# NVlabs/sionna

Measured on NVIDIA H100. Metric: coded bits/s, LDPC5G n=8448 k=4224 BP-20 decode, higher is better.
Workload: dtype f32

## Files before the change

### sionna_b200/csrc/ldpc_bp_qc.cu

```cuda
#include <algorithm>
#include <climits>
#include <iterator>
#include <numeric>
#include <vector>
#include "sb_common.h"
#include "sb_math.h"
#include "sb_math2.cuh"
#include "ldpc_graph.h"
#include "ldpc_rules.cuh"

namespace {

constexpr int kLoop = INT_MAX;
constexpr int kRowMax[] = {kLoop, 20, 12, 8, 4};
constexpr int kColCut = 7, kColFused = 10;
constexpr int kColMax[] = {kLoop, 32, 20, 12, 8, 4, 2, kLoop, 12, 4, 1};
constexpr int kRowClasses = (int)std::size(kRowMax);
constexpr int kColClasses = (int)std::size(kColMax);

constexpr bool decreasing(const int* m, int lo, int hi) {
    for (int k = lo + 1; k < hi; ++k)
        if (m[k] >= m[k - 1]) return false;
    return true;
}
static_assert(decreasing(kRowMax, 0, kRowClasses), "row class bounds must decrease");
static_assert(decreasing(kColMax, 0, kColCut) && decreasing(kColMax, kColCut, kColFused), "column class bounds must decrease");
static_assert(kColFused == kColClasses - 1 && kColMax[kColFused] == 1, "the fused class holds degree-1 columns only");

constexpr int degree_class(const int* m, int lo, int hi, int d) {
    int k = hi - 1;
    while (k > lo && d > m[k]) --k;
    return k;
}

struct QcParams {
    int Z, n_rows, n_cols, nnz, N, E, E_alloc, n_in, n_out;
    int row_cls_end[kRowClasses];
    int col_cls_end[kColClasses];
    int row_cls_mod[kRowClasses];
    int col_cls_mod[kColClasses];
    const int4* row_info;
    const int4* col_info;
    const int2* col_edge;
    const int* in_idx;
    const int* out_pos;
    const int* slot_of_edge;
    const float* llr;
    float* out;
    float* state_out;
    long long B;
    int num_iter, hard_out, use_tma;
    int early;
    int* iters_out;
    const int2* row_edge;
    int tab_rep;
    float offset, llr_max;
};


#define SB_PHI_HI 16.635532f
#define SB_PHI_ZERO 14.7117348f
template <class LT, class Probe>
__device__ __forceinline__ uint2 phi_pass1_pair(unsigned b0, unsigned b1, float& P, const LT& lt, Probe probe) {
    const float a0 = __uint_as_float(b0 & 0x7fffffffu), a1 = __uint_as_float(b1 & 0x7fffffffu);
    const float2 p = sb_phif2(make_float2(a0, a1), lt);
    probe(a0, a1);
    P = __fadd_rn(P, p.x);
    P = __fadd_rn(P, p.y);
    return make_uint2(__float_as_uint(p.x) | (b0 & 0x80000000u), __float_as_uint(p.y) | (b1 & 0x80000000u));
}
template <class LT>
__device__ __forceinline__ unsigned phi_pass1(unsigned b0, float& P, const LT& lt) {
    const float p = sb_phif_s(__uint_as_float(b0 & 0x7fffffffu), lt);
    P = __fadd_rn(P, p);
    return __float_as_uint(p) | (b0 & 0x80000000u);
}
template <class LT>
__device__ __forceinline__ uint2 phi_pass2_pair(unsigned w0, unsigned w1, float P, unsigned par, float clip, const LT& lt) {
    const float2 m = fadd2(make_float2(__uint_as_float(w0 | 0x80000000u), __uint_as_float(w1 | 0x80000000u)),
                           make_float2(P, P));
    const float2 y = sb_phif2(m, lt);
    return make_uint2(__float_as_uint(fminf(y.x, clip)) | ((w0 ^ par) & 0x80000000u),
                      __float_as_uint(fminf(y.y, clip)) | ((w1 ^ par) & 0x80000000u));
}
template <class LT>
__device__ __forceinline__ unsigned phi_pass2(unsigned w0, float P, unsigned par, float clip, const LT& lt) {
    const float y = sb_phif_s(__fadd_rn(__uint_as_float(w0 | 0x80000000u), P), lt);
    return __float_as_uint(fminf(y, clip)) | ((w0 ^ par) & 0x80000000u);
}
__device__ __forceinline__ unsigned ldw(const float* q) { return __float_as_uint(*q); }
__device__ __forceinline__ void stw(float* q, unsigned w) { *q = __uint_as_float(w); }

template <class LT>
__device__ __noinline__ void cn_phi_qc(float* pm, int Z, int deg, float clip, int* sat_flag, LT lt) {
    const unsigned am = __activemask();
    float P = 0.f;
    unsigned par = 0;
    int l = 0;
#pragma unroll 2
    for (; l + 1 < deg; l += 2) {
        float* q0 = pm + l * Z;
        float* q1 = q0 + Z;
        const unsigned b0 = ldw(q0), b1 = ldw(q1);
        par ^= b0 ^ b1;
        const uint2 w = phi_pass1_pair(b0, b1, P, lt, [&](float a0, float a1) {
            if (l == 0 && __all_sync(am, a0 >= SB_PHI_HI && a1 >= SB_PHI_HI)) *sat_flag = 1;
        });
        stw(q0, w.x);
        stw(q1, w.y);
    }
    if (l < deg) {
        float* q0 = pm + l * Z;
        const unsigned b0 = ldw(q0);
        par ^= b0;
        stw(q0, phi_pass1(b0, P, lt));
    }
    par &= 0x80000000u;
    l = 0;
#pragma unroll 2
    for (; l + 1 < deg; l += 2) {
        float* q0 = pm + l * Z;
        float* q1 = q0 + Z;
        const uint2 y = phi_pass2_pair(ldw(q0), ldw(q1), P, par, clip, lt);
        stw(q0, y.x);
        stw(q1, y.y);
    }
    if (l < deg) stw(pm + l * Z, phi_pass2(ldw(pm + l * Z), P, par, clip, lt));
}

__device__ __forceinline__ unsigned vote_sign(unsigned S, int l, unsigned par) { return ((S >> l) << 31) ^ par; }

__device__ __forceinline__ void vote_store_fast(float* pm, int Z, int deg, unsigned S, unsigned y, unsigned ylast) {
    const unsigned par = (unsigned)__popc(S) << 31;
    for (int l = 0; l < deg - 1; ++l) stw(pm + l * Z, y | vote_sign(S, l, par));
    stw(pm + (deg - 1) * Z, ylast | vote_sign(S, deg - 1, par));
}

template <class LT>
__device__ __noinline__ void cn_vote_row(float* pm, int Z, int deg, unsigned U, unsigned S, unsigned last, float clip,
                                         unsigned ylast, LT lt) {
    if (!(U & ~(1u << (deg - 1)))) {
        const float pl = sb_phif_s(__uint_as_float(last & 0x7fffffffu), lt);
        vote_store_fast(pm, Z, deg, S, __float_as_uint(fminf(sb_phif_s(pl, lt), clip)), ylast);
        return;
    }
    const unsigned par = (unsigned)__popc(S) << 31;
    float P = 0.f;
    unsigned u = U;
    for (; u & (u - 1); u &= u - 1) {
        float* q0 = pm + (__ffs(u) - 1) * Z;
        u &= u - 1;
        float* q1 = pm + (__ffs(u) - 1) * Z;
        const uint2 w = phi_pass1_pair(ldw(q0), ldw(q1), P, lt, [](float, float) {});
        stw(q0, w.x);
        stw(q1, w.y);
    }
    if (u) {
        float* q0 = pm + (__ffs(u) - 1) * Z;
        stw(q0, phi_pass1(ldw(q0), P, lt));
    }
    const unsigned rest = ~U & (0xffffffffu >> (32 - deg));
    if (rest) {
        const unsigned y = __float_as_uint(fminf(sb_phif_s(P, lt), clip));
        for (unsigned r = rest; r; r &= r - 1) {
            const int l = __ffs(r) - 1;
            stw(pm + l * Z, y | vote_sign(S, l, par));
        }
    }
    for (u = U; u & (u - 1); u &= u - 1) {
        float* q0 = pm + (__ffs(u) - 1) * Z;
        u &= u - 1;
        float* q1 = pm + (__ffs(u) - 1) * Z;
        const uint2 y = phi_pass2_pair(ldw(q0), ldw(q1), P, par, clip, lt);
        stw(q0, y.x);
        stw(q1, y.y);
    }
    if (u) {
        float* q0 = pm + (__ffs(u) - 1) * Z;
        stw(q0, phi_pass2(ldw(q0), P, par, clip, lt));
    }
}

template <int D, class LT>
__device__ __forceinline__ void cn_phi_qc_reg(float* pm, int Z, float clip, int* sat_flag, const LT& lt) {
    const unsigned am = __activemask();
    unsigned w[D];
    float P = 0.f;
    unsigned par = 0;
#pragma unroll
    for (int l = 0; l + 1 < D; l += 2) {
        const unsigned b0 = ldw(pm + l * Z), b1 = ldw(pm + (l + 1) * Z);
        par ^= b0 ^ b1;
        const uint2 q = phi_pass1_pair(b0, b1, P, lt, [&](float a0, float a1) {
            if (l == 0 && __all_sync(am, a0 >= SB_PHI_HI && a1 >= SB_PHI_HI)) *sat_flag = 1;
        });
        w[l] = q.x;
        w[l + 1] = q.y;
    }
    if (D & 1) {
        const unsigned b0 = ldw(pm + (D - 1) * Z);
        par ^= b0;
        w[D - 1] = phi_pass1(b0, P, lt);
    }
    par &= 0x80000000u;
#pragma unroll
    for (int l = 0; l + 1 < D; l += 2) {
        const uint2 y = phi_pass2_pair(w[l], w[l + 1], P, par, clip, lt);
        stw(pm + l * Z, y.x);
        stw(pm + (l + 1) * Z, y.y);
    }
    if (D & 1) stw(pm + (D - 1) * Z, phi_pass2(w[D - 1], P, par, clip, lt));
}

template <class LT, int... DS>
__device__ __forceinline__ bool cn_phi_reg_of(float* pm, int Z, int deg, float clip, int* sat_flag, const LT& lt) {
    return ((deg == DS && (cn_phi_qc_reg<DS, LT>(pm, Z, clip, sat_flag, lt), true)) || ...);
}

template <int CLS, class LT>
__device__ __forceinline__ void cn_phi_dispatch(float* pm, int Z, int deg, float clip, int* sat_flag, const LT& lt) {
    if (CLS == 4 && cn_phi_reg_of<LT, 3, 4>(pm, Z, deg, clip, sat_flag, lt)) return;
    if (CLS == 3 && cn_phi_reg_of<LT, 5, 6, 7, 8>(pm, Z, deg, clip, sat_flag, lt)) return;
    cn_phi_qc<LT>(pm, Z, deg, clip, sat_flag, lt);
}

struct StrideEdges {
    float* pm;
    int Z;
    __device__ __forceinline__ float in(int l) const { return pm[l * Z]; }
    __device__ __forceinline__ void out(int l, float v) const { pm[l * Z] = v; }
    __device__ __forceinline__ float staged(int l) const { return pm[l * Z]; }
};

__device__ __forceinline__ float2 minsum_mags(float m1, float m2, int deg, float clip, float offset) {
    float min_e = (m2 == m1) ? m1 : __fadd_rn(__fsub_rn(m2, m1), m1);
    if (deg == 1) min_e = __fadd_rn(100000.f, m1);
    return make_float2(fminf(fmaxf(__fsub_rn(m1, offset), 0.f), clip), fminf(fmaxf(__fsub_rn(min_e, offset), 0.f), clip));
}
__device__ __forceinline__ float minsum_msg(float v, float m1, float2 o, unsigned par) {
    const float mag = (fabsf(v) == m1) ? o.y : o.x;
    return __uint_as_float(__float_as_uint(mag) | ((__float_as_uint(v) ^ par) & 0x80000000u));
}
template <int DMAX, bool EXACT>
__device__ __forceinline__ void cn_minsum_qc(float* pm, int Z, int deg, float clip, float offset) {
    float x[DMAX];
    float m1 = INFINITY, m2 = INFINITY;
    unsigned par = 0;
#pragma unroll
    for (int l = 0; l < DMAX; ++l) {
        float v = INFINITY;
        if (EXACT || l < deg) v = pm[l * Z];
        x[l] = v;
        float a = fabsf(v);
        m2 = fminf(m2, fmaxf(m1, a));
        m1 = fminf(m1, a);
        par ^= __float_as_uint(v);
    }
    par &= 0x80000000u;
    const float2 o = minsum_mags(m1, m2, deg, clip, offset);
#pragma unroll
    for (int l = 0; l < DMAX; ++l) {
        const float y = minsum_msg(x[l], m1, o, par);
        if (EXACT || l < deg) pm[l * Z] = y;
    }
}

__device__ __forceinline__ void cn_minsum_qc_loop(float* pm, int Z, int deg, float clip, float offset) {
    float m1 = INFINITY, m2 = INFINITY;
    unsigned par = 0;
    for (int l = 0; l < deg; ++l) {
        float v = pm[l * Z];
        float a = fabsf(v);
        m2 = fminf(m2, fmaxf(m1, a));
        m1 = fminf(m1, a);
        par ^= __float_as_uint(v);
    }
    par &= 0x80000000u;
    const float2 o = minsum_mags(m1, m2, deg, clip, offset);
    for (int l = 0; l < deg; ++l) pm[l * Z] = minsum_msg(pm[l * Z], m1, o, par);
}

template <int RULE, int CLS, class LT>
__device__ __forceinline__ void cn_qc(float* pm, int Z, int deg, float clip, float offset, int* sat_flag, const LT& lt) {
    if constexpr (RULE == SB_CN_BOXPLUS_PHI) {
        cn_phi_dispatch<CLS, LT>(pm, Z, deg, clip, sat_flag, lt);
    } else if constexpr (RULE == SB_CN_BOXPLUS) {
        cn_tanh(StrideEdges{pm, Z}, deg, clip);
    } else {
        constexpr int D = kRowMax[CLS];
        const float off = (RULE == SB_CN_MINSUM) ? 0.f : offset;
        if constexpr (D == kLoop) {
            cn_minsum_qc_loop(pm, Z, deg, clip, off);
        } else if constexpr (CLS == 4) {
            if (deg == 3) cn_minsum_qc<3, true>(pm, Z, deg, clip, off);
            else if (deg == 4) cn_minsum_qc<4, true>(pm, Z, deg, clip, off);
            else cn_minsum_qc<D, false>(pm, Z, deg, clip, off);
        } else if constexpr (CLS == 3) {
            if (deg == 5) cn_minsum_qc<5, true>(pm, Z, deg, clip, off);
            else if (deg == 6) cn_minsum_qc<6, true>(pm, Z, deg, clip, off);
            else if (deg == 7) cn_minsum_qc<7, true>(pm, Z, deg, clip, off);
            else cn_minsum_qc<D, true>(pm, Z, deg, clip, off);
        } else if constexpr (CLS == 2) {
            if (deg == 9) cn_minsum_qc<9, true>(pm, Z, deg, clip, off);
            else if (deg == 10) cn_minsum_qc<10, true>(pm, Z, deg, clip, off);
            else cn_minsum_qc<D, false>(pm, Z, deg, clip, off);
        } else {
            if (deg == 19) cn_minsum_qc<19, true>(pm, Z, deg, clip, off);
            else cn_minsum_qc<D, false>(pm, Z, deg, clip, off);
        }
    }
}

__device__ __forceinline__ float lds_f32(uint32_t a) {
    float v;
    asm volatile("ld.shared.f32 %0, [%1];" : "=f"(v) : "r"(a));
    return v;
}
__device__ __forceinline__ void sts_f32(uint32_t a, float v) {
    asm volatile("st.shared.f32 [%0], %1;" ::"r"(a), "f"(v) : "memory");
}
__device__ __forceinline__ int2 lds_i2(uint32_t a) {
    int2 v;
    asm volatile("ld.shared.v2.s32 {%0, %1}, [%2];" : "=r"(v.x), "=r"(v.y) : "r"(a));
    return v;
}

template <int DMAX, bool CHECK, bool KEEPM, int MODE, bool EXACT = false>
__device__ __forceinline__ float vn_qc(uint32_t msg_s, uint32_t ce_s, int deg, int j4, int Z4, float llr, float clip) {
    uint32_t addr[DMAX];
    float m[KEEPM ? DMAX : 1];
    bool on[DMAX];
    float acc = 0.f;
#pragma unroll
    for (int k = 0; k < DMAX; ++k) {
        int2 e = make_int2(0, 0);
        if (EXACT || k < deg) e = lds_i2(ce_s + 8 * k);
        int t = j4 - (e.y & 0xffff);
        t += (t >> 31) & Z4;
        bool ok = EXACT || ((k < deg) && (!CHECK || t < (int)((unsigned)e.y >> 16)));
        on[k] = ok;
        addr[k] = msg_s + e.x + t;
        float v = 0.f;
        if (MODE == 0) {
            if (ok) v = lds_f32(addr[k]);
            if (ok) acc = __fadd_rn(acc, v);
        }
        if (KEEPM) m[KEEPM ? k : 0] = v;
    }
    float x_tot = __fadd_rn(acc, llr);
    const float init = __fadd_rn(llr, 0.f);
#pragma unroll
    for (int k = 0; k < DMAX; ++k) {
        if (MODE == 1) {
            if (on[k]) sts_f32(addr[k], init);
        } else {
            float v = 0.f;
            if (KEEPM) v = m[KEEPM ? k : 0];
            else if (on[k]) v = lds_f32(addr[k]);
            float y = clipf(__fadd_rn(-v, x_tot), clip);
            if (on[k]) sts_f32(addr[k], y);
        }
    }
    return x_tot;
}

template <int MODE>
__device__ __forceinline__ float vn_qc_loop(uint32_t msg_s, uint32_t ce_s, int deg, int j4, int Z4, float llr, float clip) {
    float acc = 0.f;
    if (MODE == 0)
        for (int k = 0; k < deg; ++k) {
            int2 e = lds_i2(ce_s + 8 * k);
            int t = j4 - (e.y & 0xffff);
            t += (t >> 31) & Z4;
            if (t < (int)((unsigned)e.y >> 16)) acc = __fadd_rn(acc, lds_f32(msg_s + e.x + t));
        }
    float x_tot = __fadd_rn(acc, llr);
    for (int k = 0; k < deg; ++k) {
        int2 e = lds_i2(ce_s + 8 * k);
        int t = j4 - (e.y & 0xffff);
        t += (t >> 31) & Z4;
        if (t < (int)((unsigned)e.y >> 16)) {
            uint32_t a = msg_s + e.x + t;
            sts_f32(a, (MODE == 1) ? __fadd_rn(llr, 0.f) : clipf(__fadd_rn(-lds_f32(a), x_tot), clip));
        }
    }
    return x_tot;
}

template <int MODE, int CLS, bool EX>
__device__ __forceinline__ float vn_cls(uint32_t msgb, uint32_t ce, int deg, int j4, int Z4, float llr, float clip) {
    constexpr int D = kColMax[CLS];
    if constexpr (D == kLoop) {
        return vn_qc_loop<MODE>(msgb, ce, deg, j4, Z4, llr, clip);
    } else if constexpr (CLS >= kColCut) {
        return vn_qc<D, true, true, MODE>(msgb, ce, deg, j4, Z4, llr, clip);
    } else if constexpr (D > 12) {
        return vn_qc<D, false, false, MODE>(msgb, ce, deg, j4, Z4, llr, clip);
    } else {
        if constexpr (CLS == 3) {
            if (EX && deg == 9) return vn_qc<9, false, true, MODE, true>(msgb, ce, deg, j4, Z4, llr, clip);
            if (EX && deg == 10) return vn_qc<10, false, true, MODE, true>(msgb, ce, deg, j4, Z4, llr, clip);
            if (EX && deg == 11) return vn_qc<11, false, true, MODE, true>(msgb, ce, deg, j4, Z4, llr, clip);
        } else if constexpr (CLS == 4) {
            if (EX && deg == 5) return vn_qc<5, false, true, MODE, true>(msgb, ce, deg, j4, Z4, llr, clip);
            if (EX && deg == 6) return vn_qc<6, false, true, MODE, true>(msgb, ce, deg, j4, Z4, llr, clip);
            if (EX && deg == 7) return vn_qc<7, false, true, MODE, true>(msgb, ce, deg, j4, Z4, llr, clip);
        } else if constexpr (CLS == 5) {
            if (EX && deg == 3) return vn_qc<3, false, true, MODE, true>(msgb, ce, deg, j4, Z4, llr, clip);
        } else {
            if (EX && deg == 1) return vn_qc<1, false, true, MODE, true>(msgb, ce, deg, j4, Z4, llr, clip);
        }
        return vn_qc<D, false, true, MODE, EX>(msgb, ce, deg, j4, Z4, llr, clip);
    }
}

struct WarpCtx {
    int G, grp, lane_i;
};

__device__ __forceinline__ int first_of(int start, int start_mod, const WarpCtx& w) {
    return start + (w.grp - start_mod + (w.grp < start_mod ? w.G : 0));
}

__device__ __forceinline__ void fused_vn(const QcParams& p, float* q, float c2v, int fw, int lane_i, const float* llr_s,
                                         float clip, unsigned char* hd) {
    int s = fw >> 16, vb = fw & 0xffff;
    int j = lane_i + s;
    j -= (j >= p.Z) ? p.Z : 0;
    float x_tot = __fadd_rn(__fadd_rn(0.f, c2v), llr_s[vb * p.Z + j]);
    *q = clipf(__fadd_rn(-c2v, x_tot), clip);
    if (hd) hd[vb * p.Z + j] = 0.f >= x_tot ? 1 : 0;
}

template <int RULE, int CLS, class LT>
__device__ __forceinline__ void cn_class(const QcParams& p, const WarpCtx& w, float* msg, const float* llr_s,
                                         const int4* s_row, int start, int end, float clip, bool fuse, int* sat_flag,
                                         const LT& lt, unsigned char* hd) {
    for (int rr = first_of(start, p.row_cls_mod[CLS], w); rr < end; rr += w.G) {
        int4 ri = s_row[rr];
        if (w.lane_i < ri.z) {
            float* pm = msg + ri.x * p.Z + w.lane_i;
            cn_qc<RULE, CLS, LT>(pm, p.Z, ri.y, clip, p.offset, sat_flag, lt);
            if (fuse && ri.w >= 0) {
                float* q = pm + (ri.y - 1) * p.Z;
                fused_vn(p, q, *q, ri.w, w.lane_i, llr_s, clip, hd);
            }
        }
    }
}

template <int RULE, class LT>
__device__ __forceinline__ void cn_all(const QcParams& p, const WarpCtx& w, float* msg, const float* llr_s,
                                       const int4* s_row, float clip, bool fuse, int* sat_flag, const LT& lt,
                                       unsigned char* hd) {
    const int* re = p.row_cls_end;
    cn_class<RULE, 0, LT>(p, w, msg, llr_s, s_row, 0, re[0], clip, fuse, sat_flag, lt, hd);
    cn_class<RULE, 1, LT>(p, w, msg, llr_s, s_row, re[0], re[1], clip, fuse, sat_flag, lt, hd);
    cn_class<RULE, 2, LT>(p, w, msg, llr_s, s_row, re[1], re[2], clip, fuse, sat_flag, lt, hd);
    cn_class<RULE, 3, LT>(p, w, msg, llr_s, s_row, re[2], re[3], clip, fuse, sat_flag, lt, hd);
    cn_class<RULE, 4, LT>(p, w, msg, llr_s, s_row, re[3], re[4], clip, fuse, sat_flag, lt, hd);
}

struct VoteRow {
    float* pm;
    int deg;
    bool act;
    unsigned own, S, last;
};

__device__ __forceinline__ VoteRow vote_row(float* msg, int4 ri, const WarpCtx& w, int Z) {
    VoteRow r;
    r.pm = msg + ri.x * Z + w.lane_i;
    r.deg = ri.y <= 32 ? ri.y : 0;
    r.act = w.lane_i < ri.z && r.deg > 0;
    r.own = r.S = r.last = 0;
    if (r.act) {
        r.last = ldw(r.pm + (r.deg - 1) * Z);
        r.own = fabsf(__uint_as_float(r.last)) < SB_PHI_ZERO ? 1u : 0u;
        r.S = r.last >> 31;
    }
    return r;
}

__device__ __forceinline__ void vote_read(VoteRow& r, int l, int o) {
    if (r.act && l < r.deg - 1) {
        const unsigned b = ldw(r.pm + o);
        r.own = __funnelshift_l(fabsf(__uint_as_float(b)) < SB_PHI_ZERO ? 0x80000000u : 0u, r.own, 1);
        r.S = __funnelshift_l(b, r.S, 1);
    }
}

template <class LT>
__device__ __forceinline__ void cn_vote_pass(const QcParams& p, const WarpCtx& w, float* msg, const float* llr_s,
                                             const int4* s_row, float clip, bool fuse, float phi_max, int* sat_flag,
                                             const LT& lt, unsigned char* hd) {
    const int Z = p.Z;
    const unsigned ylast = __float_as_uint(fminf(phi_max, clip));
    for (int rr = w.grp; rr < p.n_rows; rr += w.G) {
        const int4 ri = s_row[rr];
        VoteRow r = vote_row(msg, ri, w, Z);
        for (int l = r.deg - 2, o = l * Z; l >= 0; --l, o -= Z) vote_read(r, l, o);
        const unsigned U = __reduce_or_sync(0xffffffffu, r.own);
        if (r.act) cn_vote_row<LT>(r.pm, Z, r.deg, U, r.S, r.last, clip, ylast, lt);
        if (ri.y > 32 && w.lane_i < ri.z) cn_phi_qc<LT>(r.pm, Z, ri.y, clip, sat_flag, lt);
        if (fuse && ri.w >= 0 && w.lane_i < ri.z) {
            float* q = r.pm + (ri.y - 1) * Z;
            fused_vn(p, q, *q, ri.w, w.lane_i, llr_s, clip, hd);
        }
    }
}

__device__ __forceinline__ void syndrome_pass(const QcParams& p, const WarpCtx& w, const int4* s_row,
                                              const unsigned char* hd, int* unsat) {
    for (int rr = w.grp; rr < p.n_rows; rr += w.G) {
        const int4 ri = s_row[rr];
        if (w.lane_i < ri.z) {
            unsigned par = 0;
            for (int l = 0; l < ri.y; ++l) {
                const int2 e = __ldg(p.row_edge + ri.x + l);
                int j = w.lane_i + e.y;
                j -= (j >= p.Z) ? p.Z : 0;
                par ^= hd[e.x + j];
            }
            if (par) *unsat = 1;
        }
    }
}

template <int MODE, int CLS, bool EX>
__device__ __forceinline__ void vn_class(const QcParams& p, const WarpCtx& w, uint32_t msgb, const float* llr_s,
                                         const int4* s_col, uint32_t s_ce, int start, int end, float clip,
                                         bool final_pass, long long b, unsigned char* hd) {
    for (int cc = first_of(start, p.col_cls_mod[CLS], w); cc < end; cc += w.G) {
        int4 ci = s_col[cc];
        if (w.lane_i < ci.z) {
            int v = ci.w + w.lane_i;
            float x_tot = vn_cls<MODE, CLS, EX>(msgb, s_ce + 8 * ci.x, ci.y, 4 * w.lane_i, 4 * p.Z, llr_s[v], clip);
            if (MODE == 0 && hd) hd[v] = 0.f >= x_tot ? 1 : 0;
            if (MODE == 0 && final_pass) {
                int o = p.out_pos[v];
                if (o >= 0) {
                    x_tot = clipf(x_tot, clip);
                    p.out[(size_t)b * p.n_out + o] = decoder_out(x_tot, p.hard_out);
                }
            }
        }
    }
}

template <int MODE, bool EX>
__device__ __forceinline__ void vn_all(const QcParams& p, const WarpCtx& w, uint32_t msgb, const float* llr_s,
                                       const int4* s_col, uint32_t s_ce, float clip, bool final_pass,
                                       bool with_fused, long long b, unsigned char* hd = nullptr) {
    const int* ce = p.col_cls_end;
    vn_class<MODE, 0, EX>(p, w, msgb, llr_s, s_col, s_ce, 0, ce[0], clip, final_pass, b, hd);
    vn_class<MODE, 1, EX>(p, w, msgb, llr_s, s_col, s_ce, ce[0], ce[1], clip, final_pass, b, hd);
    vn_class<MODE, 2, EX>(p, w, msgb, llr_s, s_col, s_ce, ce[1], ce[2], clip, final_pass, b, hd);
    vn_class<MODE, 3, EX>(p, w, msgb, llr_s, s_col, s_ce, ce[2], ce[3], clip, final_pass, b, hd);
    vn_class<MODE, 4, EX>(p, w, msgb, llr_s, s_col, s_ce, ce[3], ce[4], clip, final_pass, b, hd);
    vn_class<MODE, 5, EX>(p, w, msgb, llr_s, s_col, s_ce, ce[4], ce[5], clip, final_pass, b, hd);
    vn_class<MODE, 6, EX>(p, w, msgb, llr_s, s_col, s_ce, ce[5], ce[6], clip, final_pass, b, hd);
    vn_class<MODE, 7, EX>(p, w, msgb, llr_s, s_col, s_ce, ce[6], ce[7], clip, final_pass, b, hd);
    vn_class<MODE, 8, EX>(p, w, msgb, llr_s, s_col, s_ce, ce[7], ce[8], clip, final_pass, b, hd);
    vn_class<MODE, 9, EX>(p, w, msgb, llr_s, s_col, s_ce, ce[8], ce[9], clip, final_pass, b, hd);
    if (with_fused) vn_class<MODE, 10, EX>(p, w, msgb, llr_s, s_col, s_ce, ce[9], ce[10], clip, final_pass, b, hd);
}

constexpr int kQcThreads = 768;

template <int RULE, int REP, bool EARLY>
__global__ void __launch_bounds__(kQcThreads, 1) ldpc_bp_qc_kernel(const __grid_constant__ QcParams p) {
    const int T = blockDim.x, tid = threadIdx.x, lane = tid & 31, warp = tid >> 5, W = T >> 5;
    const int Z = p.Z, N = p.N, Zb = (Z + 31) >> 5;
    unsigned char* const smem_raw = sb_smem + (RULE == SB_CN_BOXPLUS_PHI ? LogTab<REP>::bytes : 0);
    const int off_llr = p.E_alloc * 4;
    const int off_col = (off_llr + N * 4 + 15) & ~15;
    const int off_row = off_col + p.n_cols * 16;
    const int off_ce = off_row + p.n_rows * 16;
    const int off_bar = (off_ce + p.nnz * 8 + 15) & ~15;
    float* msg = reinterpret_cast<float*>(smem_raw);
    float* llr_s = reinterpret_cast<float*>(smem_raw + off_llr);
    int4* s_col = reinterpret_cast<int4*>(smem_raw + off_col);
    int4* s_row = reinterpret_cast<int4*>(smem_raw + off_row);
    int2* s_ce_p = reinterpret_cast<int2*>(smem_raw + off_ce);
    uint64_t* bar = reinterpret_cast<uint64_t*>(smem_raw + off_bar);
    int* sat_flag = reinterpret_cast<int*>(smem_raw + off_bar + 8);
    int* unsat = reinterpret_cast<int*>(smem_raw + off_bar + 12);
    unsigned char* hd = EARLY ? smem_raw + off_bar + 16 : nullptr;
    const uint32_t msgb = smem_u32(smem_raw);
    const uint32_t s_ce = msgb + off_ce;
    WarpCtx w;
    w.G = W / Zb;
    w.grp = warp / Zb;
    w.lane_i = (warp - w.grp * Zb) * 32 + lane;

    for (int i = tid; i < p.n_cols; i += T) s_col[i] = p.col_info[i];
    for (int i = tid; i < p.n_rows; i += T) s_row[i] = p.row_info[i];
    for (int i = tid; i < p.nnz; i += T) s_ce_p[i] = p.col_edge[i];
    const LogTab<REP> lt(lane);
    if (RULE == SB_CN_BOXPLUS_PHI) LogTab<REP>::fill(tid, T);
    if (p.use_tma && tid == 0) mbar_init(bar);
    __syncthreads();

    const float clip = p.llr_max;
    const float phi_max = sb_phif(0.f);
    uint32_t tma_phase = 0;

    for (long long b = blockIdx.x; b < p.B; b += gridDim.x) {
        load_channel_llr(llr_s, p.llr + (size_t)b * p.n_in, p.in_idx, N, p.n_in, clip, p.use_tma, msg, bar, tma_phase,
                         tid, T);
        __syncthreads();
        if (tid == 0) *sat_flag = 0;
        vn_all<1, true>(p, w, msgb, llr_s, s_col, s_ce, clip, false, true, b);
        __syncthreads();
        if (p.num_iter == 0) {
            for (int v = tid; v < N; v += T) {
                int o = p.out_pos[v];
                if (o >= 0) p.out[(size_t)b * p.n_out + o] = decoder_out(llr_s[v], p.hard_out);
            }
        }
        int limit = p.num_iter;
        for (int it = 0; it < limit; ++it) {
            if (EARLY && it > 0 && it < limit - 1) {
                if (tid == 0) *unsat = 0;
                __syncthreads();
                syndrome_pass(p, w, s_row, hd, unsat);
                __syncthreads();
                if (*unsat == 0) limit = it + 1;
            }
            const bool final_pass = it == limit - 1;
            const bool sc = *sat_flag != 0;
            if (final_pass && tid == 0 && p.use_tma && b + gridDim.x < p.B)
                asm volatile("cp.async.bulk.prefetch.L2.global [%0], %1;" ::"l"(p.llr + (size_t)(b + gridDim.x) * p.n_in),
                             "r"((uint32_t)p.n_in * 4u) : "memory");
            if constexpr (RULE == SB_CN_BOXPLUS_PHI) {
                if (sc) cn_vote_pass(p, w, msg, llr_s, s_row, clip, !final_pass, phi_max, sat_flag, lt, hd);
                else cn_all<RULE>(p, w, msg, llr_s, s_row, clip, !final_pass, sat_flag, lt, hd);
            } else {
                cn_all<RULE>(p, w, msg, llr_s, s_row, clip, !final_pass, sat_flag, lt, hd);
            }
            __syncthreads();
            vn_all<0, true>(p, w, msgb, llr_s, s_col, s_ce, clip, final_pass, final_pass, b, hd);
            __syncthreads();
        }
        if (EARLY && p.iters_out && tid == 0) p.iters_out[b] = limit;
        if (p.state_out) {
            store_state(p.state_out + (size_t)b * p.E, msg, p.slot_of_edge, p.E, tid, T);
            __syncthreads();
        }
    }
}

size_t qc_smem_bytes(const sb_ldpc_graph* g, int tab_rep, int early = 0) {
    return (early ? (size_t)g->N + 16 : 0) + ((size_t)g->qc_nnz * g->qc_Z + g->N) * 4 + 16 + (size_t)g->qc_cols * 16 + (size_t)g->qc_rows * 16 +
           (size_t)g->qc_nnz * 8 + 16 + 16 + (size_t)tab_rep * SB_LOGTAB_N * 8;
}

int qc_ensure_uploaded(sb_ldpc_graph* g) {
    if (g->qc_uploaded) return SB_OK;
    int rc;
    if ((rc = sb_upload(&g->d_qc_row_info, g->qc_row_info))) return rc;
    if ((rc = sb_upload(&g->d_qc_col_info, g->qc_col_info))) return rc;
    if ((rc = sb_upload(&g->d_qc_col_edge, g->qc_col_edge))) return rc;
    if ((rc = sb_upload(&g->d_qc_in_idx, g->qc_in_idx))) return rc;
    if ((rc = sb_upload(&g->d_qc_out_pos, g->qc_out_pos))) return rc;
    if ((rc = sb_upload(&g->d_qc_slot_of_edge, g->qc_slot_of_edge))) return rc;
    if ((rc = sb_upload(&g->d_qc_row_edge, g->qc_row_edge))) return rc;
    g->qc_uploaded = true;
    return SB_OK;
}

template <int RULE, bool EARLY>
int launch_qc(const sb_ldpc_graph* g, const QcParams& p, int threads, size_t smem, cudaStream_t stream) {
    auto kern = ldpc_bp_qc_kernel<RULE, 16, EARLY>;
    if constexpr (RULE == SB_CN_BOXPLUS_PHI) {
        if (p.tab_rep == 8) kern = ldpc_bp_qc_kernel<RULE, 8, EARLY>;
        if (p.tab_rep == 1) kern = ldpc_bp_qc_kernel<RULE, 1, EARLY>;
    }
    return sb_launch_decoder(kern, p, g, threads, smem, LLONG_MAX, stream, "sb_ldpc_decode(qc)");
}

}

void sb_qc_free_device(sb_ldpc_graph* g) {
    if (!g->qc_uploaded) return;
    cudaFree(g->d_qc_row_info); cudaFree(g->d_qc_col_info); cudaFree(g->d_qc_col_edge); cudaFree(g->d_qc_in_idx);
    cudaFree(g->d_qc_out_pos); cudaFree(g->d_qc_slot_of_edge); cudaFree(g->d_qc_row_edge);
    g->qc_uploaded = false;
}

extern "C" int sb_ldpc_graph_set_qc(sb_ldpc_graph* g, int32_t Z, int32_t n_entries, const int32_t* base_row,
                                    const int32_t* base_col, const int32_t* shift) {
    SB_CHECK_ARG(g && Z > 0 && Z <= 16383 && n_entries > 0 && base_row && base_col && shift, "sb_ldpc_graph_set_qc: bad arguments");
    SB_CHECK_ARG((int)g->h_cn.size() == g->E, "sb_ldpc_graph_set_qc: handle holds no edge list");
    SB_CHECK_ARG(!g->ref_order, "sb_ldpc_graph_set_qc: the QC kernel sums in ascending neighbour order; graphs created with "
                                "sb_ldpc_graph_create_ordered stay on the generic kernel");
    const int C = g->C, N = g->N, E = g->E;
    const int n_rows = (C + Z - 1) / Z, n_cols = (N + Z - 1) / Z;
    auto zrow = [&](int r) { return std::min(Z, C - r * Z); };
    auto zcol = [&](int c) { return std::min(Z, N - c * Z); };
    struct Ent { int r, c, s; };
    std::vector<Ent> ents;
    for (int k = 0; k < n_entries; ++k) {
        if (base_row[k] < 0 || base_col[k] < 0 || shift[k] < 0) { sb_set_error("sb_ldpc_graph_set_qc: negative entry"); return SB_EINVAL; }
        if (base_row[k] >= n_rows || base_col[k] >= n_cols) continue;
        ents.push_back({base_row[k], base_col[k], shift[k] % Z});
    }
    std::vector<long long> keys(E);
    for (int e = 0; e < E; ++e) keys[e] = ((long long)g->h_cn[e] << 32) | (unsigned)g->h_vn[e];
    std::sort(keys.begin(), keys.end());
    long long total = 0;
    for (const Ent& en : ents)
        for (int i = 0; i < zrow(en.r); ++i) {
            int j = (i + en.s) % Z;
            long long key = ((long long)(en.r * Z + i) << 32) | (unsigned)(en.c * Z + j);
            if (j >= zcol(en.c) || !std::binary_search(keys.begin(), keys.end(), key)) {
                sb_set_error("sb_ldpc_graph_set_qc: base entry (%d,%d,%d) does not match the graph", en.r, en.c, en.s);
                return SB_EINVAL;
            }
            ++total;
        }
    if (total != E) { sb_set_error("sb_ldpc_graph_set_qc: %lld lifted edges != %d graph edges", total, E); return SB_EINVAL; }
    std::vector<int> rdeg(n_rows, 0), cdeg(n_cols, 0);
    for (const Ent& en : ents) { ++rdeg[en.r]; ++cdeg[en.c]; }
    std::vector<std::vector<Ent>> by_row(n_rows), by_col(n_cols);
    for (const Ent& en : ents) { by_row[en.r].push_back(en); by_col[en.c].push_back(en); }
    for (auto& v : by_row) std::sort(v.begin(), v.end(), [](const Ent& a, const Ent& b) { return a.c < b.c; });
    for (auto& v : by_col) std::sort(v.begin(), v.end(), [](const Ent& a, const Ent& b) { return a.r < b.r; });
    std::vector<int> fused_col_of_row(n_rows, -1);
    std::vector<char> col_fused(n_cols, 0);
    for (int r = 0; r < n_rows; ++r) {
        if (by_row[r].empty()) continue;
        const Ent& last = by_row[r].back();
        if (cdeg[last.c] == 1 && rdeg[r] >= 2 && last.c < 65536 && zcol(last.c) == zrow(r)) {
            fused_col_of_row[r] = last.c;
            col_fused[last.c] = 1;
        }
    }
    auto row_class = [&](int r) { return degree_class(kRowMax, 0, kRowClasses, rdeg[r]); };
    auto col_class = [&](int c) {
        if (col_fused[c]) return kColFused;
        bool check = false;
        for (const Ent& en : by_col[c]) check = check || zrow(en.r) < Z;
        return check ? degree_class(kColMax, kColCut, kColFused, cdeg[c]) : degree_class(kColMax, 0, kColCut, cdeg[c]);
    };
    std::vector<int> rorder(n_rows), corder(n_cols);
    std::iota(rorder.begin(), rorder.end(), 0);
    std::iota(corder.begin(), corder.end(), 0);
    std::stable_sort(rorder.begin(), rorder.end(), [&](int a, int b) {
        return row_class(a) != row_class(b) ? row_class(a) < row_class(b) : rdeg[a] > rdeg[b]; });
    std::stable_sort(corder.begin(), corder.end(), [&](int a, int b) {
        return col_class(a) != col_class(b) ? col_class(a) < col_class(b) : cdeg[a] > cdeg[b]; });
    {
        const int Zb_ = (Z + 31) / 32;
        const int G = std::max(1, (kQcThreads / 32) / Zb_);
        auto balance = [&](std::vector<int>& order, const std::vector<int>& deg, auto cls_of) {
            std::vector<long long> load(G, 0);
            size_t pos = 0;
            while (pos < order.size()) {
                size_t end = pos;
                const int c = cls_of(order[pos]);
                while (end < order.size() && cls_of(order[end]) == c) ++end;
                std::vector<int> items(order.begin() + pos, order.begin() + end);
                std::stable_sort(items.begin(), items.end(), [&](int a, int b) { return deg[a] > deg[b]; });
                size_t next = 0;
                for (size_t r0 = pos; r0 < end; r0 += G) {
                    const size_t r1 = std::min(end, r0 + (size_t)G);
                    std::vector<size_t> slots;
                    for (size_t q = r0; q < r1; ++q) slots.push_back(q);
                    std::stable_sort(slots.begin(), slots.end(), [&](size_t a, size_t b) { return load[a % G] < load[b % G]; });
                    for (size_t q : slots) {
                        order[q] = items[next++];
                        load[q % G] += deg[order[q]];
                    }
                }
                pos = end;
            }
        };
        balance(rorder, rdeg, row_class);
        balance(corder, cdeg, col_class);
    }
    std::vector<int> row_cls_end(kRowClasses, 0), col_cls_end(kColClasses, 0);
    for (int r = 0; r < n_rows; ++r) for (int k = row_class(r); k < kRowClasses; ++k) ++row_cls_end[k];
    for (int c = 0; c < n_cols; ++c) for (int k = col_class(c); k < kColClasses; ++k) ++col_cls_end[k];
    std::vector<int> be_of((size_t)n_rows * n_cols, -1);
    std::vector<int> row_info(4 * n_rows), row_edge;
    int be = 0;
    for (int rr = 0; rr < n_rows; ++rr) {
        int r = rorder[rr];
        row_info[4 * rr] = be;
        row_info[4 * rr + 1] = rdeg[r];
        row_info[4 * rr + 2] = zrow(r);
        row_info[4 * rr + 3] = fused_col_of_row[r] >= 0 ? (fused_col_of_row[r] | (by_row[r].back().s << 16)) : -1;
        for (const Ent& en : by_row[r]) {
            if (be_of[(size_t)en.r * n_cols + en.c] != -1) { sb_set_error("sb_ldpc_graph_set_qc: duplicate base entry"); return SB_EINVAL; }
            be_of[(size_t)en.r * n_cols + en.c] = be++;
            row_edge.push_back(en.c * Z);
            row_edge.push_back(en.s);
        }
    }
    const int nnz = be;
    std::vector<int> col_info(4 * n_cols), col_edge(2 * (size_t)nnz);
    int ce = 0;
    for (int cc = 0; cc < n_cols; ++cc) {
        int c = corder[cc];
        col_info[4 * cc] = ce;
        for (const Ent& en : by_col[c]) {
            col_edge[2 * ce] = be_of[(size_t)en.r * n_cols + en.c] * Z * 4;
            col_edge[2 * ce + 1] = (en.s * 4) | ((zrow(en.r) * 4) << 16);
            ++ce;
        }
        col_info[4 * cc + 1] = cdeg[c];
        col_info[4 * cc + 2] = zcol(c);
        col_info[4 * cc + 3] = c * Z;
    }
    std::vector<int> in_nat(N), out_nat(N), slot(E);
    for (int r = 0; r < N; ++r) { in_nat[g->vn_order[r]] = g->in_idx[r]; out_nat[g->vn_order[r]] = g->out_pos[r]; }
    for (int e = 0; e < E; ++e) {
        int r = g->h_cn[e] / Z, i = g->h_cn[e] % Z, c = g->h_vn[e] / Z;
        slot[e] = be_of[(size_t)r * n_cols + c] * Z + i;
    }
    sb_qc_free_device(g);
    g->qc = true; g->qc_Z = Z; g->qc_rows = n_rows; g->qc_cols = n_cols; g->qc_nnz = nnz;
    g->qc_max_row_deg = *std::max_element(rdeg.begin(), rdeg.end());
    g->qc_max_col_deg = *std::max_element(cdeg.begin(), cdeg.end());
    g->qc_row_info.swap(row_info); g->qc_col_info.swap(col_info); g->qc_col_edge.swap(col_edge);
    g->qc_row_cls_end = row_cls_end; g->qc_col_cls_end = col_cls_end;
    g->qc_in_idx.swap(in_nat); g->qc_out_pos.swap(out_nat); g->qc_slot_of_edge.swap(slot); g->qc_row_edge.swap(row_edge);
    return SB_OK;
}

namespace {
__global__ void debug_phi_kernel(const float* x, float* o1, float* o2, long long n) {
    LogTab<16>::fill(threadIdx.x, blockDim.x);
    __syncthreads();
    const LogTab<16> lt(threadIdx.x & 31);
    long long i = (long long)blockIdx.x * blockDim.x + threadIdx.x;
    if (2 * i + 1 < n) {
        float2 r = sb_phif2(make_float2(x[2 * i], x[2 * i + 1]), lt);
        o2[2 * i] = r.x; o2[2 * i + 1] = r.y;
        o1[2 * i] = sb_phif(x[2 * i]); o1[2 * i + 1] = sb_phif(x[2 * i + 1]);
    }
}
}
extern "C" int sb_debug_phi(const float* d_x, float* d_scalar, float* d_packed, int64_t n, void* stream) {
    if (n == 0) return SB_OK;
    SB_CHECK_ARG(d_x && d_scalar && d_packed && n >= 0 && n % 2 == 0, "sb_debug_phi: bad arguments");
    debug_phi_kernel<<<(unsigned)((n / 2 + 255) / 256), 256, LogTab<16>::bytes, (cudaStream_t)stream>>>(d_x, d_scalar,
                                                                                                         d_packed, n);
    SB_LAUNCH_CHECK();
    return SB_OK;
}

extern "C" int sb_ldpc_graph_is_qc(const sb_ldpc_graph* g) { return g && g->qc ? 1 : 0; }

int sb_qc_try_decode(sb_ldpc_graph* g, const float* d_llr, int64_t batch, int32_t num_iter, int32_t cn_rule,
                     int32_t vn_rule, float offset, float llr_max, int32_t hard_out, const float* d_state_in,
                     float* d_state_out, float* d_out, cudaStream_t stream, bool* handled, int32_t early, int32_t* d_iters) {
    *handled = false;
    if (!g->qc || !g->flooding || vn_rule != SB_VN_SUM || d_state_in || cn_rule > SB_CN_OFFSET_MINSUM) return SB_OK;
    int tab_rep = cn_rule == SB_CN_BOXPLUS_PHI ? 16 : 0;
    if (tab_rep && qc_smem_bytes(g, tab_rep, early) > (size_t)g->smem_optin) tab_rep = 8;
    if (tab_rep && qc_smem_bytes(g, tab_rep, early) > (size_t)g->smem_optin) tab_rep = 1;
    const size_t smem = qc_smem_bytes(g, tab_rep, early);
    if (smem > (size_t)g->smem_optin) return SB_OK;
    if ((cn_rule == SB_CN_MINSUM || cn_rule == SB_CN_OFFSET_MINSUM) &&
        !(llr_max < 100000.f && (float)(g->qc_max_row_deg - 1) * llr_max < 99000.f))
        return SB_OK;
    int rc = qc_ensure_uploaded(g);
    if (rc) return rc;
    QcParams p{};
    p.Z = g->qc_Z; p.n_rows = g->qc_rows; p.n_cols = g->qc_cols; p.nnz = g->qc_nnz; p.N = g->N; p.E = g->E;
    p.E_alloc = g->qc_nnz * g->qc_Z; p.n_in = g->n_in; p.n_out = g->n_out;
    for (int k = 0; k < kRowClasses; ++k) p.row_cls_end[k] = g->qc_row_cls_end[k];
    for (int k = 0; k < kColClasses; ++k) p.col_cls_end[k] = g->qc_col_cls_end[k];
    p.row_info = (const int4*)g->d_qc_row_info; p.col_info = (const int4*)g->d_qc_col_info;
    p.col_edge = (const int2*)g->d_qc_col_edge; p.in_idx = g->d_qc_in_idx; p.out_pos = g->d_qc_out_pos;
    p.slot_of_edge = g->d_qc_slot_of_edge;
    p.llr = d_llr; p.out = d_out; p.state_out = d_state_out; p.B = batch; p.num_iter = num_iter; p.hard_out = hard_out;
    p.offset = offset; p.llr_max = llr_max; p.tab_rep = tab_rep;
    p.early = early; p.iters_out = d_iters; p.row_edge = (const int2*)g->d_qc_row_edge;
    p.use_tma = (g->n_in % 4 == 0) && (g->n_in <= p.E_alloc) && ((reinterpret_cast<uintptr_t>(d_llr) & 15) == 0);
    const int Zb = (g->qc_Z + 31) / 32;
    const int max_warps = kQcThreads / 32;
    int groups = std::max(1, std::min(max_warps / Zb, std::max(g->qc_rows, g->qc_cols)));
    const int threads = groups * Zb * 32;
    for (int k = 0; k < kRowClasses; ++k) p.row_cls_mod[k] = (k ? g->qc_row_cls_end[k - 1] : 0) % groups;
    for (int k = 0; k < kColClasses; ++k) p.col_cls_mod[k] = (k ? g->qc_col_cls_end[k - 1] : 0) % groups;
    rc = sb_dispatch<SB_CN_BOXPLUS_PHI, SB_CN_OFFSET_MINSUM>(cn_rule, [&](auto R) {
        return p.early ? launch_qc<R, true>(g, p, threads, smem, stream) : launch_qc<R, false>(g, p, threads, smem, stream);
    });
    *handled = (rc == SB_OK);
    return rc;
}
```

### sionna_b200/csrc/sb_math2.cuh

```cuda
#pragma once
#include "sb_math.h"

__device__ __forceinline__ int f2i_mov(float x) { int r; asm("mov.b32 %0, %1;" : "=r"(r) : "f"(x)); return r; }
__device__ __forceinline__ float i2f_mov(int x) { float r; asm("mov.b32 %0, %1;" : "=f"(r) : "r"(x)); return r; }
__device__ __forceinline__ float2 f2(float a, float b) { return make_float2(a, b); }
__device__ __forceinline__ float2 f2s(float a) { return make_float2(a, a); }
__device__ __forceinline__ float2 ffma2(float2 a, float2 b, float2 c) {
    return make_float2(__fmaf_rn(a.x, b.x, c.x), __fmaf_rn(a.y, b.y, c.y));
}
__device__ __forceinline__ float2 fadd2(float2 a, float2 b) { return make_float2(__fadd_rn(a.x, b.x), __fadd_rn(a.y, b.y)); }
__device__ __forceinline__ float2 fmul2(float2 a, float2 b) { return make_float2(__fmul_rn(a.x, b.x), __fmul_rn(a.y, b.y)); }

__device__ __forceinline__ float2 sb_expf2_inrange(float2 x) {
    float2 t = ffma2(x, f2s(1.44269504088896341f), f2s(12582912.0f));
    float2 nf = fadd2(t, f2s(-12582912.0f));
    float2 r = ffma2(nf, f2s(-0.693145751953125f), x);
    r = ffma2(nf, f2s(-1.42860677e-06f), r);
    float2 g = ffma2(f2s(0x1.a124e4p-13f), r, f2s(0x1.6d4316p-10f));
    g = ffma2(g, r, f2s(0x1.1110e0p-7f));
    g = ffma2(g, r, f2s(0x1.5554eap-5f));
    g = ffma2(g, r, f2s(0x1.555556p-3f));
    g = ffma2(g, r, f2s(0.5f));
    float2 r2 = fmul2(r, r);
    float2 s = ffma2(r2, g, r);
    float2 p = fadd2(f2s(1.0f), s);
    return f2(i2f_mov((int)((unsigned)f2i_mov(p.x) + ((unsigned)f2i_mov(t.x) << 23))),
              i2f_mov((int)((unsigned)f2i_mov(p.y) + ((unsigned)f2i_mov(t.y) << 23))));
}

__device__ __forceinline__ float2 sb_logf2(float2 y) {
    int ix0 = f2i_mov(y.x), ix1 = f2i_mov(y.y);
    int e0 = (ix0 - 0x3f3504f3) >> 23, e1 = (ix1 - 0x3f3504f3) >> 23;
    float2 m = f2(i2f_mov(ix0 - (e0 << 23)), i2f_mov(ix1 - (e1 << 23)));
    float2 ef = f2((float)e0, (float)e1);
    float2 r = fadd2(m, f2s(-1.0f));
    float2 p = ffma2(f2s(0x1.1d8ea6p-4f), r, f2s(-0x1.d635bcp-4f));
    p = ffma2(p, r, f2s(0x1.dea282p-4f));
    p = ffma2(p, r, f2s(-0x1.fcf4c6p-4f));
    p = ffma2(p, r, f2s(0x1.23d21ap-3f));
    p = ffma2(p, r, f2s(-0x1.555b4ap-3f));
    p = ffma2(p, r, f2s(0x1.999d5ap-3f));
    p = ffma2(p, r, f2s(-0x1.fffffcp-3f));
    p = ffma2(p, r, f2s(0x1.555554p-2f));
    float2 r2 = fmul2(r, r);
    float2 r3 = fmul2(r2, r);
    float2 nh = fmul2(f2s(-0.5f), r2);
    float2 tl = ffma2(r3, p, nh);
    float2 lo = ffma2(ef, f2s(1.42860677e-06f), tl);
    float2 t2 = fadd2(r, lo);
    return ffma2(ef, f2s(0.693145751953125f), t2);
}

extern __shared__ __align__(16) unsigned char sb_smem[];

template <int REP>
struct LogTab {
    uint32_t lane_off;
    static constexpr int bytes = SB_LOGTAB_N * REP * 8;
    static constexpr int log_stride = REP == 16 ? 7 : (REP == 8 ? 6 : 3);
    static constexpr int rs = SB_LOGTAB_SHIFT - log_stride;
    static constexpr int mask = (SB_LOGTAB_N - 1) << log_stride;
    __device__ static void fill(int tid, int T) {
        float2* tab = reinterpret_cast<float2*>(sb_smem);
        for (int i = tid; i < SB_LOGTAB_N * REP; i += T)
            tab[i] = make_float2(sb_logtab_dev[2 * (i / REP)], sb_logtab_dev[2 * (i / REP) + 1]);
    }
    __device__ explicit LogTab(int lane) : lane_off(8 * (lane & (REP - 1))) {}
};

template <int MASK>
__device__ __forceinline__ int and_or(int a, int c) {
    int d;
    asm("lop3.b32 %0, %1, %2, %3, 0xEA;" : "=r"(d) : "r"(a), "n"(MASK), "r"(c));
    return d;
}

template <class LT>
__device__ __forceinline__ float2 logtab_entry(int ix, const LT& lt) {
    float2 v;
    asm("ld.shared.v2.f32 {%0, %1}, [%2];" : "=f"(v.x), "=f"(v.y)
        : "r"((uint32_t)__cvta_generic_to_shared(sb_smem) + and_or<LT::mask>(ix >> LT::rs, lt.lane_off)));
    return v;
}

__device__ __forceinline__ float logtab_expf(int ix) { return i2f_mov((int)(((unsigned)ix >> 23) + 0x4B400000u)); }

template <class LT>
__device__ __forceinline__ float2 sb_logf2_tab(float2 y, const LT& lt) {
    int ix0 = f2i_mov(y.x), ix1 = f2i_mov(y.y);
    float2 c0 = logtab_entry(ix0, lt), c1 = logtab_entry(ix1, lt);
    float2 inv_c = f2(c0.x, c1.x);
    float2 logc = f2(c0.y, c1.y);
    float2 m = f2(i2f_mov(and_or<0x007fffff>(ix0, 0x3f800000)), i2f_mov(and_or<0x007fffff>(ix1, 0x3f800000)));
    float2 F = f2(logtab_expf(ix0), logtab_expf(ix1));
    float2 ef = fadd2(F, f2s(-12583039.0f));
    float2 r = ffma2(m, inv_c, f2s(-1.0f));
    float2 q = ffma2(r, f2s(-0.25f), f2s(0x1.555556p-2f));
    q = ffma2(q, r, f2s(-0.5f));
    float2 r2 = fmul2(r, r);
    float2 s = ffma2(r2, q, r);
    float2 lo = ffma2(ef, f2s(1.42860677e-06f), s);
    float2 t2 = fadd2(logc, lo);
    return ffma2(ef, f2s(0.693145751953125f), t2);
}

template <class LT>
__device__ __forceinline__ float sb_logf_tab_s(float y, const LT& lt) {
    int ix = __float_as_int(y);
    float2 c = logtab_entry(ix, lt);
    return sb_logf_tab_core(ix, c.x, c.y);
}

template <class LT>
__device__ __forceinline__ float2 sb_phif2(float2 x, const LT& lt) {
    x.x = fminf(fmaxf(x.x, 8.5e-8f), 16.635532f);
    x.y = fminf(fmaxf(x.y, 8.5e-8f), 16.635532f);
    float2 t = sb_expf2_inrange(x);
    float2 la = sb_logf2_tab(fadd2(t, f2s(1.0f)), lt);
    float2 lb = sb_logf2_tab(fadd2(t, f2s(-1.0f)), lt);
    return ffma2(lb, f2s(-1.0f), la);
}

template <class LT>
__device__ __forceinline__ float sb_phif_s(float x, const LT& lt) {
    x = fminf(fmaxf(x, 8.5e-8f), 16.635532f);
    float t = sb_expf(x);
    return __fsub_rn(sb_logf_tab_s(__fadd_rn(t, 1.0f), lt), sb_logf_tab_s(__fadd_rn(t, -1.0f), lt));
}
```

Measured before the change: 2.749 billion.

## Restructure vote check-node pass with shared-memory address loads and inline fast path

Rewrites the vote-based check-node pass so that reads of each row go through explicit shared-memory addresses, two at a time, and the unsatisfied-bit test becomes a subtract plus sign bit. The all-satisfied fast path moves inline, calling phi twice inside a loop that is not unrolled and writing signs from a shifted mask. The check-to-variable value is kept in a register for the fused variable-node update instead of being re-read. The scalar phi now uses a branchless in-range exp, which relies on the input clamp. This adds code complexity and a small risk of sign or ordering mistakes in exchange for fewer instructions per row.

Result: faster. 2.935 billion (median of 6 runs) (+6.7%).

```diff
diff --git a/sionna_b200/csrc/ldpc_bp_qc.cu b/sionna_b200/csrc/ldpc_bp_qc.cu
--- a/sionna_b200/csrc/ldpc_bp_qc.cu
+++ b/sionna_b200/csrc/ldpc_bp_qc.cu
@@ -130,20 +130,8 @@
 
 __device__ __forceinline__ unsigned vote_sign(unsigned S, int l, unsigned par) { return ((S >> l) << 31) ^ par; }
 
-__device__ __forceinline__ void vote_store_fast(float* pm, int Z, int deg, unsigned S, unsigned y, unsigned ylast) {
-    const unsigned par = (unsigned)__popc(S) << 31;
-    for (int l = 0; l < deg - 1; ++l) stw(pm + l * Z, y | vote_sign(S, l, par));
-    stw(pm + (deg - 1) * Z, ylast | vote_sign(S, deg - 1, par));
-}
-
 template <class LT>
-__device__ __noinline__ void cn_vote_row(float* pm, int Z, int deg, unsigned U, unsigned S, unsigned last, float clip,
-                                         unsigned ylast, LT lt) {
-    if (!(U & ~(1u << (deg - 1)))) {
-        const float pl = sb_phif_s(__uint_as_float(last & 0x7fffffffu), lt);
-        vote_store_fast(pm, Z, deg, S, __float_as_uint(fminf(sb_phif_s(pl, lt), clip)), ylast);
-        return;
-    }
+__device__ __noinline__ void cn_vote_row(float* pm, int Z, int deg, unsigned U, unsigned S, float clip, LT lt) {
     const unsigned par = (unsigned)__popc(S) << 31;
     float P = 0.f;
     unsigned u = U;
@@ -461,52 +449,77 @@
     cn_class<RULE, 4, LT>(p, w, msg, llr_s, s_row, re[3], re[4], clip, fuse, sat_flag, lt, hd);
 }
 
-struct VoteRow {
-    float* pm;
-    int deg;
-    bool act;
-    unsigned own, S, last;
-};
-
-__device__ __forceinline__ VoteRow vote_row(float* msg, int4 ri, const WarpCtx& w, int Z) {
-    VoteRow r;
-    r.pm = msg + ri.x * Z + w.lane_i;
-    r.deg = ri.y <= 32 ? ri.y : 0;
-    r.act = w.lane_i < ri.z && r.deg > 0;
-    r.own = r.S = r.last = 0;
-    if (r.act) {
-        r.last = ldw(r.pm + (r.deg - 1) * Z);
-        r.own = fabsf(__uint_as_float(r.last)) < SB_PHI_ZERO ? 1u : 0u;
-        r.S = r.last >> 31;
-    }
-    return r;
-}
-
-__device__ __forceinline__ void vote_read(VoteRow& r, int l, int o) {
-    if (r.act && l < r.deg - 1) {
-        const unsigned b = ldw(r.pm + o);
-        r.own = __funnelshift_l(fabsf(__uint_as_float(b)) < SB_PHI_ZERO ? 0x80000000u : 0u, r.own, 1);
-        r.S = __funnelshift_l(b, r.S, 1);
-    }
+__device__ __forceinline__ unsigned unsat_bit31(unsigned b) {
+    return __float_as_uint(__fadd_rn(fabsf(__uint_as_float(b)), -SB_PHI_ZERO));
 }
 
 template <class LT>
 __device__ __forceinline__ void cn_vote_pass(const QcParams& p, const WarpCtx& w, float* msg, const float* llr_s,
                                              const int4* s_row, float clip, bool fuse, float phi_max, int* sat_flag,
                                              const LT& lt, unsigned char* hd) {
-    const int Z = p.Z;
+    const int Z = p.Z, Z4 = 4 * Z;
+    const int msgb = (int)smem_u32(msg);
     const unsigned ylast = __float_as_uint(fminf(phi_max, clip));
     for (int rr = w.grp; rr < p.n_rows; rr += w.G) {
         const int4 ri = s_row[rr];
-        VoteRow r = vote_row(msg, ri, w, Z);
-        for (int l = r.deg - 2, o = l * Z; l >= 0; --l, o -= Z) vote_read(r, l, o);
-        const unsigned U = __reduce_or_sync(0xffffffffu, r.own);
-        if (r.act) cn_vote_row<LT>(r.pm, Z, r.deg, U, r.S, r.last, clip, ylast, lt);
-        if (ri.y > 32 && w.lane_i < ri.z) cn_phi_qc<LT>(r.pm, Z, ri.y, clip, sat_flag, lt);
-        if (fuse && ri.w >= 0 && w.lane_i < ri.z) {
-            float* q = r.pm + (ri.y - 1) * Z;
-            fused_vn(p, q, *q, ri.w, w.lane_i, llr_s, clip, hd);
-        }
+        const bool act = w.lane_i < ri.z;
+        float c2v = 0.f;
+        if (ri.y > 32) {
+            if (act) {
+                float* pm = msg + ri.x * Z + w.lane_i;
+                cn_phi_qc<LT>(pm, Z, ri.y, clip, sat_flag, lt);
+                c2v = pm[(ri.y - 1) * Z];
+            }
+        } else if (ri.y > 0) {
+            const int deg = ri.y;
+            const int a0 = msgb + 4 * (ri.x * Z + (act ? w.lane_i : 0));
+            const int top = a0 + (deg - 1) * Z4;
+            const unsigned last = __float_as_uint(lds_f32(top));
+            unsigned own = unsat_bit31(last) >> 31, S = last >> 31;
+            int a = top - Z4;
+            if (!(deg & 1)) {
+                const unsigned b = __float_as_uint(lds_f32(a));
+                own = __funnelshift_l(unsat_bit31(b), own, 1);
+                S = __funnelshift_l(b, S, 1);
+                a -= Z4;
+            }
+            for (; a > a0; a -= 2 * Z4) {
+                const unsigned b1 = __float_as_uint(lds_f32(a)), b0 = __float_as_uint(lds_f32(a - Z4));
+                own = __funnelshift_l(unsat_bit31(b1), own, 1);
+                own = __funnelshift_l(unsat_bit31(b0), own, 1);
+                S = __funnelshift_l(b1, S, 1);
+                S = __funnelshift_l(b0, S, 1);
+            }
+            const unsigned U = __reduce_or_sync(0xffffffffu, act ? own : 0u);
+            if (!(U & ~(1u << (deg - 1)))) {
+                float y = __uint_as_float(last & 0x7fffffffu);
+#pragma unroll 1
+                for (int k = 0; k < 2; ++k) y = sb_phif_s(y, lt);
+                if (act) {
+                    const unsigned yb = __float_as_uint(fminf(y, clip));
+                    unsigned v = (S ^ (0u - (__popc(S) & 1u))) << (32 - deg);
+                    const unsigned wl = ylast | (v & 0x80000000u);
+                    sts_f32(top, __uint_as_float(wl));
+                    c2v = __uint_as_float(wl);
+                    int a = top - Z4;
+                    if (!(deg & 1)) {
+                        v <<= 1;
+                        sts_f32(a, __uint_as_float(yb | (v & 0x80000000u)));
+                        a -= Z4;
+                    }
+                    for (; a > a0; a -= 2 * Z4) {
+                        sts_f32(a, __uint_as_float(yb | ((v << 1) & 0x80000000u)));
+                        sts_f32(a - Z4, __uint_as_float(yb | ((v << 2) & 0x80000000u)));
+                        v <<= 2;
+                    }
+                }
+            } else if (act) {
+                cn_vote_row<LT>(msg + ri.x * Z + w.lane_i, Z, deg, U, S, clip, lt);
+                c2v = lds_f32(top);
+            }
+        }
+        if (fuse && ri.w >= 0 && act)
+            fused_vn(p, msg + (ri.x + ri.y - 1) * Z + w.lane_i, c2v, ri.w, w.lane_i, llr_s, clip, hd);
     }
 }
 
diff --git a/sionna_b200/csrc/sb_math2.cuh b/sionna_b200/csrc/sb_math2.cuh
--- a/sionna_b200/csrc/sb_math2.cuh
+++ b/sionna_b200/csrc/sb_math2.cuh
@@ -26,6 +26,21 @@
     float2 p = fadd2(f2s(1.0f), s);
     return f2(i2f_mov((int)((unsigned)f2i_mov(p.x) + ((unsigned)f2i_mov(t.x) << 23))),
               i2f_mov((int)((unsigned)f2i_mov(p.y) + ((unsigned)f2i_mov(t.y) << 23))));
+}
+
+__device__ __forceinline__ float sb_expf_inrange(float x) {
+    float t = __fmaf_rn(x, 1.44269504088896341f, 12582912.0f);
+    float nf = __fadd_rn(t, -12582912.0f);
+    float r = __fmaf_rn(nf, -0.693145751953125f, x);
+    r = __fmaf_rn(nf, -1.42860677e-06f, r);
+    float g = __fmaf_rn(0x1.a124e4p-13f, r, 0x1.6d4316p-10f);
+    g = __fmaf_rn(g, r, 0x1.1110e0p-7f);
+    g = __fmaf_rn(g, r, 0x1.5554eap-5f);
+    g = __fmaf_rn(g, r, 0x1.555556p-3f);
+    g = __fmaf_rn(g, r, 0.5f);
+    float s = __fmaf_rn(__fmul_rn(r, r), g, r);
+    float p = __fadd_rn(1.0f, s);
+    return i2f_mov((int)((unsigned)f2i_mov(p) + ((unsigned)f2i_mov(t) << 23)));
 }
 
 __device__ __forceinline__ float2 sb_logf2(float2 y) {
@@ -124,6 +139,6 @@
 template <class LT>
 __device__ __forceinline__ float sb_phif_s(float x, const LT& lt) {
     x = fminf(fmaxf(x, 8.5e-8f), 16.635532f);
-    float t = sb_expf(x);
+    float t = sb_expf_inrange(x);
     return __fsub_rn(sb_logf_tab_s(__fadd_rn(t, 1.0f), lt), sb_logf_tab_s(__fadd_rn(t, -1.0f), lt));
 }
```
